# ducha-aiki/mods

Measured on AMD Instinct MI355X. Metric: image-pairs/sec (1024x768, HessAff+RootSIFT over the affine view ladder, MFMA FGINN match, LO-RANSAC H), higher is better.
Workload: dtype f32 (detect/describe) + u8 on the int8 matrix cores (distance matrix)

## Files before the change

include/modsx.h:

```cpp
#ifndef MODSX_H
#define MODSX_H
#include <stdint.h>
#ifdef __cplusplus
extern "C" {
#endif

#define MODSX_VERSION 100

typedef enum modsx_status {
  MODSX_OK = 0,
  MODSX_ERR_ARG = -1,
  MODSX_ERR_DEVICE = -2,
  MODSX_ERR_NOMEM = -3,
  MODSX_ERR_INTERNAL = -4,
  MODSX_ERR_CAPACITY = -5,
  MODSX_ERR_TIMEOUT = -6
} modsx_status;

enum { MODSX_FIXED_TH = 0, MODSX_RELATIVE_TH = 1, MODSX_FIXED_REG_NUMBER = 2, MODSX_RELATIVE_REG_NUMBER = 3,
       MODSX_NOT_LESS_THAN_REGIONS = 4 };
enum { MODSX_DET_HESSIAN = 0, MODSX_DET_DOG = 1, MODSX_DET_HARRIS = 2, MODSX_DET_MSER = 3 };
enum { MODSX_DESC_SIFT = 0, MODSX_DESC_ROOT_SIFT = 1, MODSX_DESC_HALF_SIFT = 2, MODSX_DESC_HALF_ROOT_SIFT = 3 };
#define MODSX_MAX_DESC 4
enum { MODSX_HESSIAN_DARK = 0, MODSX_HESSIAN_BRIGHT = 1, MODSX_HESSIAN_SADDLE = 2 };
// ... 178 lines not shown
                     const modsx_pair_params *par, modsx_pair_result *res);
void modsx_pair_result_release(modsx_pair_result *res);

int modsx_match_pairs(modsx_ctx *const *ctxs, int n_ctx, const modsx_image *const *imgs1,
                      const modsx_image *const *imgs2, int n_pairs, const modsx_pair_params *par,
                      modsx_pair_result *results);

int modsx_match_pairs_views(modsx_ctx *const *ctxs, int n_ctx, const modsx_image *const *imgs1,
                            const modsx_image *const *imgs2, int n_pairs, const modsx_view *views, int n_views,
                            const modsx_pair_params *par, modsx_pair_result *results);

int modsx_last_batch_verify(double *sum_ms, int *pairs, int *threads);
int modsx_last_match_geometry(int *qs, int *fat, int *S, int *tiles_per_split, int *ntiles_ub);
int modsx_describe_counters(modsx_ctx *ctx, long *out, int n);
int modsx_blur_geometry(const int *rows, const int *cols, int n, int *geometry);
int modsx_detect_counters(modsx_ctx *ctx, long *out, int n);
int modsx_debug_pyramids(modsx_ctx *ctx, const modsx_image *const *imgs, int n, const modsx_hessaff_params *par, int *geometry,
                         float *planes, unsigned long long cap_floats, unsigned long long *need_floats);
int modsx_debug_scan_levels(modsx_ctx *ctx, const float *resps, const float *blurs, int L, int rows, int cols,
                            const modsx_hessaff_params *par, modsx_candidate **cands, int *n_cands, modsx_sskp **out);
int modsx_debug_detect_scalespace_batch(modsx_ctx *ctx, const modsx_image *const *imgs, int n, const modsx_hessaff_params *par,
                                        modsx_sskp **out, int *counts);
int modsx_debug_orientation_counts(unsigned long long *launched, unsigned long long *skipped, int reset);
int modsx_debug_orientation_launches(unsigned long long *lds_table, unsigned long long *global_table, int reset);
int modsx_orientation_tables(unsigned char *bin_table, unsigned short *index_raster, float *weight_raster,
                             unsigned short *index_lanes, float *weight_lanes, int *counts);
int modsx_debug_reproject_certain_drop(const modsx_region *regs, int n, const double *H, int orig_w, int orig_h, double boxk,
                                       unsigned char *drop);
int modsx_debug_describe_plan(const modsx_region *regs, const int *counts, int nimages, double mr_size, int fast_extraction,
                              unsigned long long arena_floats, long *counters, int n, long *cuts, int cap_cuts, int *n_cuts);
// ... 233 lines not shown
```

mods_amd/__init__.py:

```python
import ctypes as C
import os
import subprocess

import numpy as np

_HERE = os.path.dirname(os.path.abspath(__file__))
LIB_PATH = os.environ.get("MODSX_LIB", os.path.join(_HERE, "libmodsx.so"))

KEYPOINT = np.dtype([("x", "f8"), ("y", "f8"), ("a11", "f8"), ("a12", "f8"), ("a21", "f8"), ("a22", "f8"),
                     ("s", "f8"), ("response", "f8"), ("octave_number", "i4"), ("pyramid_scale", "f8"),
                     ("sub_type", "i4")], align=True)
REGION = np.dtype([("img_id", "i4"), ("img_reproj_id", "i4"), ("id", "i4"), ("parent_id", "i4"), ("type", "i4"),
                   ("det_kp", KEYPOINT), ("reproj_kp", KEYPOINT)], align=True)
SSKP = np.dtype([("octave", "i4"), ("level", "i4"), ("r0", "i4"), ("c0", "i4"), ("r", "i4"), ("c", "i4"),
                 ("type", "i4"), ("pad", "i4"), ("b0", "f4"), ("b1", "f4"), ("b2", "f4"), ("val", "f4"),
                 ("x", "f4"), ("y", "f4"), ("s", "f4"), ("pixelDistance", "f4")], align=True)
TENT = np.dtype([("q", "i4"), ("t0", "i4"), ("tj", "i4"), ("t1", "i4"), ("d1", "f8"), ("d2", "f8"),
                 ("d2by2ndcl", "f8"), ("ratio", "f8")], align=True)
CANDIDATE = np.dtype([("img", "i4"), ("octave", "i4"), ("level", "i4"), ("type", "i4"), ("r0", "i4"), ("c0", "i4"), ("r", "i4"),
                      ("c", "i4"), ("b0", "f4"), ("b1", "f4"), ("b2", "f4"), ("val", "f4")], align=True)


class HessAffParams(C.Structure):
    _fields_ = [("threshold", C.c_float), ("mode", C.c_int), ("reg_number", C.c_int),
# ... 78 lines not shown
           "modsx_view_block_order", "modsx_detect_describe_views_sharded", "modsx_match_fginn_sharded",
           "modsx_match_pair_views_sharded", "modsx_match_pairs_views_sharded", "modsx_match_ladder_sharded", "modsx_comm_loopback_id", "modsx_comm_set_lanes",
           "modsx_comm_attach", "modsx_comm_lane_done", "modsx_comm_reset_lanes", "modsx_comm_set_timeout", "modsx_comm_stats",
           "modsx_shard_block_bytes", "modsx_shard_block_pack", "modsx_shard_blocks_unpack", "modsx_shard_device_pack",
           "modsx_shard_device_unpack", "modsx_verify_device_stats", "modsx_verify_device_timing", "modsx_comm_set_exchange",
           "modsx_shard_owner_plan", "modsx_db_create", "modsx_db_free", "modsx_db_rows", "modsx_db_nearest",
           "modsx_match_fginn_db", "modsx_match_fginn_db_device", "modsx_set_fginn_db",
           "modsx_debug_orientation_counts", "modsx_debug_orientation_launches", "modsx_orientation_tables",
           "modsx_debug_reproject_certain_drop", "modsx_debug_describe_plan",
           "modsx_debug_baumberg_geometry", "modsx_debug_baumberg_geometry_ctx", "modsx_debug_baumberg_variant",
           "modsx_debug_baumberg", "modsx_debug_check_borders", "modsx_debug_describe_lanes", "modsx_debug_describe_lane_map",
           "modsx_rep_create", "modsx_rep_free", "modsx_rep_add_views", "modsx_rep_append", "modsx_rep_class",
           "modsx_rep_match_fginn", "modsx_match_reps", "modsx_match_one_to_many",
           "modsx_match_hamming", "modsx_match_hamming_device", "modsx_hamming_tentatives", "modsx_debug_match_hamming",
           "modsx_match_regions_hamming", "modsx_debug_hamming_geometry",
           "modsx_blur_geometry", "modsx_detect_counters", "modsx_debug_pyramids", "modsx_debug_scan_levels",
           "modsx_debug_detect_scalespace_batch",
           "modsx_match_fginn_f32", "modsx_match_fginn_f32_device", "modsx_match_regions_f32", "modsx_debug_match_fginn_f32",
           "modsx_debug_fginn32_geometry", "modsx_debug_fginn32_dpass",
           "modsx_extract_patches", "modsx_extract_patches_device", "modsx_liop_patches", "modsx_liop_patches_device",
           "modsx_describe_regions_liop", "modsx_describe_regions_liop_device", "modsx_liop_tables", "modsx_debug_liop",
           "modsx_liop_counters",
           "modsx_describe_regions_raw", "modsx_describe_regions_raw_device", "modsx_sift_norm_rows", "modsx_sift_norm_rows_device",
           "modsx_describe_regions_dspsift", "modsx_describe_regions_dspsift_device", "modsx_dsp_counters",
           "modsx_surf_patches", "modsx_surf_patches_device", "modsx_describe_regions_surf", "modsx_describe_regions_surf_device",
           "modsx_surf_tables", "modsx_surf_counters",
           "modsx_detect_surf", "modsx_detect_surf_batch", "modsx_surf_regions", "modsx_surfdet_geometry", "modsx_surfdet_normalise",
           "modsx_debug_surfdet", "modsx_surfdet_counters",
           "modsx_daisy_dim", "modsx_daisy_patches", "modsx_daisy_patches_device", "modsx_describe_regions_daisy",
           "modsx_describe_regions_daisy_device", "modsx_daisy_tables", "modsx_daisy_counters"]
EXPORTS_DEGENSAC = ["exp_ransacHcustom", "exp_ransacFcustom", "HDs", "HDsi", "HDsidx", "HDsSym", "HDsiSym", "HDsSymidx",
# ... 68 lines not shown
        L.modsx_db_create.restype = C.c_void_p
        L.modsx_db_create.argtypes = [C.c_void_p, C.c_void_p, C.c_long, C.c_int]
        L.modsx_db_free.restype = None
        L.modsx_db_free.argtypes = [C.c_void_p, C.c_void_p]
        L.modsx_db_rows.restype = C.c_long
        L.modsx_db_rows.argtypes = [C.c_void_p]
        L.modsx_db_nearest.argtypes = [C.c_void_p, C.c_void_p, C.c_void_p, C.c_int, C.c_void_p]
        L.modsx_set_fginn_db.argtypes = [C.c_void_p, C.c_void_p]
        L.modsx_debug_reproject_certain_drop.argtypes = [C.c_void_p, C.c_int, C.c_void_p, C.c_int, C.c_int, C.c_double, C.c_void_p]
        L.modsx_describe_counters.argtypes = [C.c_void_p, C.c_void_p, C.c_int]
        L.modsx_debug_orientation_counts.argtypes = [C.c_void_p, C.c_void_p, C.c_int]
        L.modsx_debug_orientation_launches.argtypes = [C.c_void_p, C.c_void_p, C.c_int]
        L.modsx_orientation_tables.argtypes = [C.c_void_p] * 6
        L.modsx_blur_geometry.argtypes = [C.c_void_p, C.c_void_p, C.c_int, C.c_void_p]
        L.modsx_detect_counters.argtypes = [C.c_void_p, C.c_void_p, C.c_int]
        L.modsx_debug_pyramids.argtypes = [C.c_void_p, C.c_void_p, C.c_int, C.c_void_p, C.c_void_p, C.c_void_p, C.c_ulonglong,
                                           C.c_void_p]
        L.modsx_debug_scan_levels.argtypes = [C.c_void_p, C.c_void_p, C.c_void_p, C.c_int, C.c_int, C.c_int, C.c_void_p,
                                              C.c_void_p, C.c_void_p, C.c_void_p]
        L.modsx_debug_detect_scalespace_batch.argtypes = [C.c_void_p, C.c_void_p, C.c_int, C.c_void_p, C.c_void_p, C.c_void_p]
        L.modsx_debug_describe_plan.argtypes = [C.c_void_p, C.c_void_p, C.c_int, C.c_double, C.c_int, C.c_ulonglong, C.c_void_p, C.c_int,
                                                C.c_void_p, C.c_int, C.c_void_p]
        L.modsx_debug_baumberg_geometry.argtypes = [C.c_int, C.c_int, C.c_int, C.c_int, C.c_void_p]
        L.modsx_debug_baumberg.argtypes = [C.c_void_p, C.c_void_p, C.c_int, C.c_void_p, C.c_void_p, C.c_int, C.c_void_p, C.c_int, C.c_int,
                                           C.c_void_p, C.c_void_p, C.c_void_p, C.c_void_p, C.c_void_p]
        L.modsx_debug_baumberg_variant.argtypes = [C.c_int]
        L.modsx_debug_baumberg_geometry_ctx.argtypes = [C.c_void_p, C.c_int, C.c_int, C.c_int, C.c_int, C.c_void_p]
        L.modsx_debug_check_borders.argtypes = [C.c_void_p, C.c_int, C.c_void_p]
        L.modsx_debug_describe_lanes.argtypes = [C.c_int, C.c_void_p]
        L.modsx_debug_describe_lane_map.argtypes = [C.c_int, C.c_int, C.c_void_p, C.c_void_p, C.c_int]
# ... 460 lines not shown
        return C.c_void_p(self.h)

    def upload(self, pixels):
        a = np.ascontiguousarray(pixels)
        if a.dtype == np.uint8:
            dtype = 0
        else:
            a = np.ascontiguousarray(a, np.float32)
            dtype = 1
        ch = 1 if a.ndim == 2 else a.shape[2]
        h = lib().modsx_image_upload(self._c(), _p(a), a.shape[0], a.shape[1], ch, dtype)
        if not h:
            raise RuntimeError("modsx_image_upload failed: " + _err())
        return Image(self, h, a.shape[0], a.shape[1])

    def wrap_device(self, dev_ptr, rows, cols):
        h = lib().modsx_image_wrap_device(self._c(), C.c_void_p(dev_ptr), rows, cols)
        if not h:
            raise RuntimeError("modsx_image_wrap_device failed: " + _err())
        return Image(self, h, rows, cols)

    def synchronize(self):
        _check(lib().modsx_synchronize(self._c()), "synchronize")

    def gaussian_blur(self, img, sigma):
        out = np.empty((img.rows, img.cols), np.float32)
        _check(lib().modsx_gaussian_blur(self._c(), C.c_void_p(img.h), C.c_float(sigma), _p(out)), "gaussian_blur")
        return out

    def response(self, img, detector_type, norm):
# ... 253 lines not shown
        if out_ptr is not None:
            _check(lib().modsx_describe_regions_dspsift_device(*args, C.c_void_p(out_ptr)), "describe_regions_dspsift_device")
            return None
        desc = np.zeros((len(regs), 128), np.float32)
        _check(lib().modsx_describe_regions_dspsift(*args, _p(desc)), "describe_regions_dspsift")
        return desc

    def dsp_counters(self):
        return self._counters("modsx_dsp_counters", DSP_COUNTERS)

    def describe_counters(self):
        return self._counters("modsx_describe_counters", DESCRIBE_COUNTERS)

    def detect_counters(self):
        return self._counters("modsx_detect_counters", DETECT_COUNTERS)

    def debug_pyramids(self, images, params):
        n, L = len(images), params.numberOfScales + 2
        ptrs = (C.c_void_p * max(1, n))(*[im.h for im in images])
        geo = np.zeros((max(1, n), 49), np.int32)
        need = C.c_ulonglong(0)
        _check(lib().modsx_debug_pyramids(self._c(), ptrs, n, C.byref(params), _p(geo), None, 0, C.byref(need)), "debug_pyramids")
        planes = np.empty(max(1, need.value), np.float32)
        _check(lib().modsx_debug_pyramids(self._c(), ptrs, n, C.byref(params), _p(geo), _p(planes), need.value, C.byref(need)),
               "debug_pyramids")
        out, at = [], 0
        for i in range(n):
            octs = []
            for o in range(int(geo[i, 0])):
                r, c = int(geo[i, 1 + 2 * o]), int(geo[i, 2 + 2 * o])
# ... 364 lines not shown
def hamming_tentatives(nn2, distance_threshold):
    nn2 = np.ascontiguousarray(nn2, np.int32).reshape(-1, 4)
    out = C.c_void_p()
    n = _check(lib().modsx_hamming_tentatives(_p(nn2), len(nn2), C.c_double(distance_threshold), C.byref(out)), "hamming_tentatives")
    return _take(out, n, TENT)


def blur_geometry(shapes):
    sh = np.ascontiguousarray(shapes, np.int32).reshape(-1, 2)
    rows, cols = np.ascontiguousarray(sh[:, 0]), np.ascontiguousarray(sh[:, 1])
    geo = np.zeros(2, np.int32)
    _check(lib().modsx_blur_geometry(_p(rows), _p(cols), len(sh), _p(geo)), "blur_geometry")
    return int(geo[0]), int(geo[1])


FGINN32_GEOMETRY = ("tile", "splits", "workgroups", "DK", "tiles", "tiles_per_split")


def _f32_rows(d1, d2):
    d1, d2 = np.ascontiguousarray(d1, np.float32), np.ascontiguousarray(d2, np.float32)
    if d1.ndim != 2 or d2.ndim != 2 or d1.shape[1] != d2.shape[1]:
        raise ValueError("fginn_f32: two [n][dim] arrays of one width are expected")
    return d1, d2, d1.shape[1]


def fginn32_geometry(n1, n2, dim, splits=0):
    geo = np.zeros(6, np.int32)
    _check(lib().modsx_debug_fginn32_geometry(int(n1), int(n2), int(dim), int(splits), _p(geo)), "fginn32_geometry")
    return dict(zip(FGINN32_GEOMETRY, (int(x) for x in geo)))

# ... 270 lines not shown
```

mods_amd/csrc/capi.hip:

```cpp
#include <math.h>
#include <malloc.h>
#include <algorithm>
#include <atomic>
#include <chrono>
#include <mutex>
#include <thread>
#include <condition_variable>
#include <deque>
#include "engine_api.hpp"
#include "describe_plan.hpp"
#include "describe_lanes.hpp"

using namespace mx;

#define NEED(c)                                             \
  do {                                                      \
    if (!(c)) { mx::set_error("null argument: " #c); return MODSX_ERR_ARG; } \
  } while (0)

template <typename T>
static T *to_malloc(const std::vector<T> &v) {
  T *p = (T *)malloc(sizeof(T) * (v.size() ? v.size() : 1));
  if (p && !v.empty()) memcpy(p, v.data(), sizeof(T) * v.size());
  return p;
}

// ... 111 lines not shown
int modsx_image_update(modsx_ctx *ctx, modsx_image *im, const void *pixels, int rows, int cols, int channels, int dtype) {
  NEED(ctx); NEED(im); NEED(pixels);
  if ((channels != 1 && channels != 3) || (dtype != 0 && dtype != 1) || !im->owned || rows != im->rows || cols != im->cols) {
    mx::set_error("modsx_image_update: bad argument (the image must be an uploaded one of the same size)");
    return MODSX_ERR_ARG;
  }
  hipSetDevice(ctx->dev);
  const size_t n = (size_t)rows * cols, inBytes = n * channels * (dtype == 0 ? 1 : 4);
  if (!ctx->misc.ensure(inBytes)) return MODSX_ERR_NOMEM;
  if (hipMemcpyAsync(ctx->misc.p, pixels, inBytes, hipMemcpyHostToDevice, ctx->stream) != hipSuccess) { mx::set_error("image H2D copy failed"); return MODSX_ERR_DEVICE; }
  launch_gray(ctx->stream, ctx->misc.p, im->d, n, channels, dtype);
  if (hipStreamSynchronize(ctx->stream) != hipSuccess) { mx::set_error("image update sync failed"); return MODSX_ERR_DEVICE; }
  return MODSX_OK;
}

modsx_image *modsx_image_wrap_device(modsx_ctx *ctx, const float *dev_pixels, int rows, int cols) {
  if (!ctx || !dev_pixels || rows <= 0 || cols <= 0) { mx::set_error("modsx_image_wrap_device: bad argument"); return nullptr; }
  if (!image_size_ok(rows, cols)) return nullptr;
  modsx_image *im = new modsx_image();
  im->d = const_cast<float *>(dev_pixels); im->rows = rows; im->cols = cols; im->owned = false;
  return im;
}

void modsx_image_free(modsx_ctx *ctx, modsx_image *img) {
  if (!img) return;
  if (ctx) hipSetDevice(ctx->dev);
  if (img->owned && img->d) hipFree(img->d);
  delete img;
}

// ... 52 lines not shown
  if (!ctx->scratchA.ensure(npx * 4)) return MODSX_ERR_NOMEM;
  BlurBatch b;
  memset(&b, 0, sizeof b);
  int n = blur_ksize(sigma);
  if (n > MAX_TAPS) { mx::set_error("modsx_gaussian_blur: ksize > 17"); return MODSX_ERR_ARG; }
  if (n == 1) {
    MX_HIP(hipMemcpyAsync(out, img->d, npx * 4, hipMemcpyDeviceToHost, ctx->stream));
    MX_HIP(hipStreamSynchronize(ctx->stream));
    return MODSX_OK;
  }
  std::vector<float> k = gaussian_kernel(n, sigma);
  b.n = n;
  for (int i = 0; i < n; i++) b.k[i] = k[i];
  b.j[0].src = img->d; b.j[0].blur = (float *)ctx->scratchA.p; b.j[0].resp = nullptr; b.j[0].rows = img->rows;
  b.j[0].cols = img->cols; b.j[0].norm = 1.f;
  mx::book_blur(ctx, launch_blur_hess(ctx->stream, b, 1, img->rows, img->cols));
  MX_HIP(hipMemcpyAsync(out, ctx->scratchA.p, npx * 4, hipMemcpyDeviceToHost, ctx->stream));
  MX_HIP(hipStreamSynchronize(ctx->stream));
  MX_HIP(hipGetLastError());
  return MODSX_OK;
}

static int blur_any(modsx_ctx *c, const float *src, float *dst, float *tmp, float *dTaps, float *hTaps, int rows, int cols, float sigma) {
  const int n = blur_ksize(sigma);
  if (n == 1) { MX_HIP(hipMemcpyAsync(dst, src, (size_t)rows * cols * 4, hipMemcpyDeviceToDevice, c->stream)); return MODSX_OK; }
  const int nx = cols == 1 ? 1 : n, ny = rows == 1 ? 1 : n;
  std::vector<float> kx = gaussian_kernel(nx, sigma), ky = gaussian_kernel(ny, sigma);
  memcpy(hTaps, kx.data(), nx * 4); memcpy(hTaps + nx, ky.data(), ny * 4);
  MX_HIP(hipMemcpyAsync(dTaps, hTaps, (size_t)(nx + ny) * 4, hipMemcpyHostToDevice, c->stream));
  launch_blur_pass(c->stream, src, tmp, rows, cols, dTaps, nx, 0, 1);
  launch_blur_pass(c->stream, tmp, dst, rows, cols, dTaps + nx, ny, 1, 1);
// ... 201 lines not shown
  NEED(ctx);
  if (n < 0 || (n > 0 && !out)) { mx::set_error("modsx_describe_counters: bad argument"); return MODSX_ERR_ARG; }
  long sum[mx::DC_N] = {0};
  for (const modsx_ctx *head : {(const modsx_ctx *)ctx, (const modsx_ctx *)ctx->peer})
    for (const modsx_ctx *c = head; c; c = c->half)
      for (int q = 0; q < mx::DC_N; q++)
        if (q == mx::DC_MAX_CHUNKS) sum[q] = std::max(sum[q], c->descCnt[q]); else sum[q] += c->descCnt[q];
  for (int q = 0; q < n && q < mx::DC_N; q++) out[q] = sum[q];
  return mx::DC_N;
}

int modsx_blur_geometry(const int *rows, const int *cols, int n, int *geometry) {
  NEED(rows); NEED(cols); NEED(geometry);
  if (n < 1 || n > mx::MAXB) { mx::set_error("modsx_blur_geometry: 1 .. 32 planes"); return MODSX_ERR_ARG; }
  for (int i = 0; i < n; i++)
    if (rows[i] < 1 || cols[i] < 1 || !image_size_ok(rows[i], cols[i])) { mx::set_error("modsx_blur_geometry: plane size"); return MODSX_ERR_ARG; }
  const mx::BlurGeo g = mx::blur_geometry(rows, cols, n);
  geometry[0] = g.th; geometry[1] = g.tiles;
  return MODSX_OK;
}

int modsx_detect_counters(modsx_ctx *ctx, long *out, int n) {
  NEED(ctx);
  if (n < 0 || (n > 0 && !out)) { mx::set_error("modsx_detect_counters: bad argument"); return MODSX_ERR_ARG; }
  long sum[mx::DT_N] = {0};
  for (const modsx_ctx *head : {(const modsx_ctx *)ctx, (const modsx_ctx *)ctx->peer})
    for (const modsx_ctx *c = head; c; c = c->half)
      for (int q = 0; q < mx::DT_N; q++)
        if (q != mx::DT_LAST_JOBS && q != mx::DT_LAST_TILES && q != mx::DT_LAST_ACCEPTED) sum[q] += c->detCnt[q];
  for (int q : {(int)mx::DT_LAST_JOBS, (int)mx::DT_LAST_TILES, (int)mx::DT_LAST_ACCEPTED}) sum[q] = ctx->detCnt[q];
  for (int q = 0; q < n && q < mx::DT_N; q++) out[q] = sum[q];
  return mx::DT_N;
}
// ... 1213 lines not shown
```

mods_amd/csrc/engine.hpp:

```cpp
#pragma once
#include <hip/hip_runtime.h>
#include <stdint.h>
#include <stdlib.h>
#include <string.h>
#include <string>
#include <vector>
#include "../../include/modsx.h"
#include "kmath.hpp"

namespace mx {

#ifndef MODSX_MAXB
#define MODSX_MAXB 32
#endif
constexpr int MAXB = MODSX_MAXB;
constexpr int PAIR_GROUP = 4;
constexpr int NMS_MAXJ = 1024;
constexpr int MAX_TAPS = 17;

struct BlurJob {
  const float *src;
  float *blur;
  float *resp;
  int rows, cols;
  float norm;
  int pad;
};
struct BlurBatch {
  int n;
  float k[MAX_TAPS];
  BlurJob j[MAXB];
  int nj;
  int tile0[MAXB + 1];
};
struct ResizeJob {
  const float *src;
  float *dst;
  float *resp;
  int srows, scols, drows, dcols;
  float norm;
  int pad;
};
struct ResizeBatch { ResizeJob j[MAXB]; int nj; int tile0[MAXB + 1]; };
struct NmsJob {
  const float *low, *cur, *high, *blur;
  int rows, cols, img, octave, level, pad;
};
struct NmsBatch {
// ... 122 lines not shown
  } while (0)

std::vector<float> gaussian_kernel(int n, double sigma);
int blur_ksize(float sigma);
void gauss_mask(float *mask, int size);
void circular_gauss_mask(float *mask, int size, float sigma);
const double *atan_lut_host();
inline bool check_borders_host(int w, int h, float ofsx, float ofsy, float a11, float a12, float a21, float a22, int rw, int rh) {
  return check_borders(w, h, ofsx, ofsy, a11, a12, a21, a22, rw, rh);
}
bool invert3(const double *S, double *t);
void rectify(double &a11, double &a12, double &a21, double &a22);

struct BlurGeo { int th, tiles; };
BlurGeo blur_geometry(const int *rows, const int *cols, int n);
struct BlurLaunch { int th, tiles, R; };
BlurLaunch launch_blur_hess(hipStream_t s, const BlurBatch &b, int nj, int maxRows, int maxCols);
bool launch_hessian(hipStream_t s, const BlurBatch &b, int nj, int maxRows, int maxCols);
bool launch_resize_half(hipStream_t s, const ResizeBatch &b, int nj, int maxRows, int maxCols);
void launch_nms(hipStream_t s, const NmsBatch &b, const NmsJob *jobs, const int *tilePrefix, const int *tileJob, int nj,
                int nTiles, int4 *queue, unsigned *qcount, unsigned qcap, Candidate *out, unsigned *counter, unsigned cap,
                const int *octFirst = nullptr, int levelsPerOctave = 0);
size_t cand_sort_temp_bytes(unsigned nsort);
int launch_cand_order(hipStream_t s, const Candidate *cand, const unsigned *counter, unsigned nsort, unsigned long long *keys,
                      unsigned long long *keys2, unsigned *idx, unsigned *idx2, void *temp, size_t tempBytes, unsigned long long *tabKey,
                      unsigned *tabRank, unsigned tabSize, unsigned *slotOf, Candidate *out, unsigned *outCount);
constexpr int NMS_QUEUES = 64;
constexpr int NMS_TILE_ROWS = 16;
void launch_gray(hipStream_t s, const void *src, float *dst, size_t n, int channels, int dtype);
struct BaumGeo { int kernel, chunk, nchunks, grid; };
BaumGeo baumberg_geometry(int n, int W, int variant, int chunk, int resident = 0);
// ... 208 lines not shown
  unsigned short *dOriIdx = nullptr;
  float *dSiftMask = nullptr;
  unsigned short *dSiftMaskIdx = nullptr;
  int nSiftMask = 0;
  double *dAtan = nullptr;
  unsigned char *dOriBinTab = nullptr;
  float *dSiftOTab = nullptr;
  int *dSiftBins = nullptr;
  double *dSiftW = nullptr;
  double timings[6];
  mx::Profiler prof;
  size_t lastCandCount = 0;
  const mx::DbSet *fginnDb = nullptr;
  long descCnt[mx::DC_N] = {0};
  long detCnt[mx::DT_N] = {0};
  double hammingMs[2] = {0, 0};
  double fginn32Ms[2] = {0, 0};
  mx::DevBuf patchBuf, patchOut;
  mx::DevBuf liopTab, liopDbg, liopCnt;
  long liopCounters[4] = {0, 0, 0, 0};
  mx::DevBuf dspRows;
  long dspCounters[3] = {0, 0, 0};
  static constexpr int SURF_TABS = 4;
  mx::DevBuf surfTab[SURF_TABS];
  double surfTabMr[SURF_TABS] = {0, 0, 0, 0};
  int surfTabNext = 0;
  long surfCounters[3] = {0, 0, 0};
  static constexpr int DAISY_TABS = 4;
  mx::DevBuf daisyTab[DAISY_TABS];
  int daisyTabKey[DAISY_TABS] = {0, 0, 0, 0};
  int daisyTabNext = 0;
  long daisyCounters[3] = {0, 0, 0};
  mx::DevBuf sdInteg, sdResp, sdLap, sdFlags, sdCounts, sdTab, sdPoints, sdExt;
  mx::PinBuf sdHost, sdBack;
  long sdCounters[5] = {0, 0, 0, 0, 0};
  int busyDepth = 0;
  int shardLane = 0;
  modsx_ctx *peer = nullptr;
  modsx_ctx *half = nullptr;
  mx::DevBuf halfDesc[4];
  void *worker = nullptr;
};

namespace mx {
inline void book_blur(modsx_ctx *c, const BlurLaunch &g) {
  if (!g.th) return;
  c->detCnt[g.th == 32 ? DT_BLUR_TH32 : DT_BLUR_TH16]++;
  c->detCnt[DT_BLUR_R1 + g.R - 1]++;
}
}
```

mods_amd/csrc/engine_detect.hip:

```cpp
#include <math.h>
#include <algorithm>
#include <mutex>
#include <dlfcn.h>
#include <string>
#include "engine_api.hpp"

namespace mx {

static int cv_round(double v) { return (int)lrint(v); }

struct SigmaPlan {
  int levels;
  float sigmaStep;
  float curSigma[8];
  float incSigma[8];
};

static SigmaPlan make_sigma_plan(const modsx_hessaff_params &p) {
  SigmaPlan s;
  s.levels = p.numberOfScales + 2;
  s.sigmaStep = powf(2.0f, 1.0f / (float)p.numberOfScales);
  float cur = p.initialSigma;
  s.curSigma[0] = cur; s.incSigma[0] = 0;
  for (int i = 1; i < s.levels; i++) {
// ... 68 lines not shown
    float sigma = sqrtf(p.initialSigma * p.initialSigma - curSigma0 * curSigma0);
    int rc = fill_taps(bb, sigma);
    if (rc) return rc;
  }
  for (int k = 0; k < lv.n; k++) {
    const int i = lv.img[k];
    Octave &oc = c->pyr[i].oct[0];
    BlurJob &j = bb.j[k];
    j.src = imgs[i]->d; j.blur = oc.blur[0]; j.resp = hess ? oc.resp[0] : nullptr; j.rows = oc.rows; j.cols = oc.cols;
    j.norm = sp.curSigma[0] * sp.curSigma[0];
    if (!preBlur) {
      MX_HIP(hipMemcpyAsync(oc.blur[0], imgs[i]->d, (size_t)oc.rows * oc.cols * 4, hipMemcpyDeviceToDevice, s));
      j.src = oc.blur[0];
    }
  }
  if (preBlur) { ProfScope ps(c, K_BLUR_HESS, lv.px * 12); book_blur(c, launch_blur_hess(s, bb, lv.n, lv.mr, lv.mc)); }
  else if (hess) { ProfScope ps(c, K_HESSIAN, lv.px * 8); c->detCnt[DT_HESSIAN] += launch_hessian(s, bb, lv.n, lv.mr, lv.mc); }
  return MODSX_OK;
}

static void launch_resize_level(modsx_ctx *c, const LiveOctave &lv, int o, const modsx_hessaff_params &p, const SigmaPlan &sp, bool hess) {
  ResizeBatch rb;
  memset(&rb, 0, sizeof rb);
  double spx = 0;
  for (int k = 0; k < lv.n; k++) {
    Octave &pv = c->pyr[lv.img[k]].oct[o - 1], &oc = c->pyr[lv.img[k]].oct[o];
    ResizeJob &r = rb.j[k];
    r.src = pv.blur[p.numberOfScales]; r.dst = oc.blur[0];
    r.srows = pv.rows; r.scols = pv.cols; r.drows = oc.rows; r.dcols = oc.cols;
    r.resp = hess ? oc.resp[0] : nullptr; r.norm = sp.curSigma[0] * sp.curSigma[0];
    spx += (double)pv.rows * pv.cols;
// ... 50 lines not shown
      }
    }
  }
  return MODSX_OK;
}

int build_pyramids(modsx_ctx *c, const modsx_image *const *imgs, int n, const modsx_hessaff_params &p,
                   bool singleOctaveFromFirstLevel) {
  if (n <= 0 || n > MAXB) { set_error("batch size"); return MODSX_ERR_ARG; }
  if (p.numberOfScales < 1 || p.numberOfScales > 6) { set_error("numberOfScales"); return MODSX_ERR_ARG; }
  if (p.border < 1) { set_error("border must be at least 1"); return MODSX_ERR_ARG; }
  if (p.detectorType != MODSX_DET_HESSIAN && p.detectorType != MODSX_DET_DOG && p.detectorType != MODSX_DET_HARRIS) {
    set_error("detectorType must be Hessian (0), DoG (1) or Harris (2)");
    return MODSX_ERR_ARG;
  }
  const bool hess = p.detectorType == MODSX_DET_HESSIAN;
  const SigmaPlan sp = make_sigma_plan(p);
  int maxOct = 0;
  int rc = plan_octaves(c, imgs, n, sp.levels, 2 * p.border + 2, singleOctaveFromFirstLevel, &maxOct);
  if (rc) return rc;
  for (int o = 0; o < maxOct; o++) {
    const LiveOctave lv = live_octave(c, n, o);
    if (o == 0) rc = launch_first_level(c, imgs, lv, p, sp, hess, singleOctaveFromFirstLevel);
    else launch_resize_level(c, lv, o, p, sp, hess);
    if (rc) return rc;
    for (int l = 1; l < sp.levels; l++) {
      BlurBatch b2;
      memset(&b2, 0, sizeof b2);
      rc = fill_taps(b2, sp.incSigma[l]);
      if (rc) return rc;
      for (int k = 0; k < lv.n; k++) {
        Octave &oc = c->pyr[lv.img[k]].oct[o];
        BlurJob &j = b2.j[k];
        j.src = oc.blur[l - 1]; j.blur = oc.blur[l]; j.resp = hess ? oc.resp[l] : nullptr; j.rows = oc.rows; j.cols = oc.cols;
        j.norm = sp.curSigma[l] * sp.curSigma[l];
      }
      ProfScope ps(c, K_BLUR_HESS, lv.px * 12);
      book_blur(c, launch_blur_hess(c->stream, b2, lv.n, lv.mr, lv.mc));
    }
    if (!hess) rc = launch_other_responses(c, lv, o, p, sp);
    if (rc) return rc;
  }
  MX_HIP(hipGetLastError());
  return MODSX_OK;
}

static const unsigned CAND_CAP = 1u << 21;

static NmsBatch nms_thresholds(const modsx_hessaff_params &p) {
  NmsBatch nb;
  memset(&nb, 0, sizeof nb);
  nb.edgeScoreThreshold = (p.edgeEigenValueRatio + 1.0f) * (p.edgeEigenValueRatio + 1.0f) / p.edgeEigenValueRatio;
  float finalTh = p.threshold;
// ... 520 lines not shown
```

mods_amd/csrc/kernels_pyramid.hip:

```cpp
#include "engine.hpp"

namespace mx {

constexpr int TW = 64;
constexpr int TMP_W = TW + 4;

MX_D int find_job(const int *tile0, int nj, int t) {
  int j = 0;
  while (j + 1 < nj && t >= tile0[j + 1]) j++;
  return j;
}

typedef float f2 __attribute__((ext_vector_type(2)));

template <int R, int TH>
__global__ __launch_bounds__(256) void k_blur_hess(BlurBatch batch) {
  constexpr int BLR_H = TH + 4;
  const int ji = find_job(batch.tile0, batch.nj, blockIdx.x);
  const BlurJob jb = batch.j[ji];
  const int rows = jb.rows, cols = jb.cols;
  const int lt = blockIdx.x - batch.tile0[ji], ntx = (cols + TW - 1) / TW;
  const int tx0 = (lt % ntx) * TW, ty0 = (lt / ntx) * TH;
  constexpr int n = 2 * R + 1;
  constexpr int sh = BLR_H + 2 * R, sw = TMP_W + 2 * R;
// ... 71 lines not shown
    const float *B = blr + (ly + 1) * TMP_W + (lx + 1);
    const unsigned gofs = __umul24((unsigned)gy, (unsigned)cols) + (unsigned)gx;
    jb.blur[gofs] = B[0];
    if (jb.resp) {
      float o = 0.f;
      if (gy >= 1 && gy < rows - 1 && gx >= 1 && gx < cols - 1) {
        const float v11 = B[-TMP_W - 1], v12 = B[-TMP_W], v13 = B[-TMP_W + 1];
        const float v21 = B[-1], v22 = B[0], v23 = B[1];
        const float v31 = B[TMP_W - 1], v32 = B[TMP_W], v33 = B[TMP_W + 1];
        float Lxx = (v21 - 2 * v22 + v23);
        float Lyy = (v12 - 2 * v22 + v32);
        float Lxy = (v13 - v11 + v31 - v33) / 4.0f;
        o = (Lxx * Lyy - Lxy * Lxy) * norm2;
      }
      jb.resp[gofs] = o;
    }
  }
}

__global__ __launch_bounds__(256) void k_hessian(BlurBatch batch) {
  const int ji = find_job(batch.tile0, batch.nj, blockIdx.x);
  const BlurJob jb = batch.j[ji];
  const int rows = jb.rows, cols = jb.cols;
  const int lt = blockIdx.x - batch.tile0[ji], ntx = (cols + 63) / 64;
  const int gx = (lt % ntx) * 64 + (threadIdx.x & 63), gy = (lt / ntx) * 4 + (threadIdx.x >> 6);
  if (gx >= cols || gy >= rows) return;
  float o = 0.f;
  if (gy >= 1 && gy < rows - 1 && gx >= 1 && gx < cols - 1) {
    const float *B = jb.src + (size_t)gy * cols + gx;
    const float v11 = B[-cols - 1], v12 = B[-cols], v13 = B[-cols + 1];
// ... 355 lines not shown
    case 6: hipLaunchKernelGGL((k_blur_hess<6, TH>), grid, dim3(256), 0, s, b); break;
    case 7: hipLaunchKernelGGL((k_blur_hess<7, TH>), grid, dim3(256), 0, s, b); break;
    default: hipLaunchKernelGGL((k_blur_hess<8, TH>), grid, dim3(256), 0, s, b); break;
  }
}
BlurGeo blur_geometry(const int *rows, const int *cols, int n) {
  auto tiles = [&](int th) {
    int t = 0;
    for (int i = 0; i < n; i++) t += ((cols[i] + TW - 1) / TW) * ((rows[i] + th - 1) / th);
    return t;
  };
  const int t32 = tiles(32);
  if (t32 >= 2560) return {32, t32};
  return {16, tiles(16)};
}
BlurLaunch launch_blur_hess(hipStream_t s, const BlurBatch &bin, int nj, int, int) {
  BlurBatch b = bin;
  int rows[MAXB], cols[MAXB];
  for (int i = 0; i < nj; i++) { rows[i] = b.j[i].rows; cols[i] = b.j[i].cols; }
  const BlurGeo g = blur_geometry(rows, cols, nj);
  if (g.tiles <= 0) return {0, 0, 0};
  const int tiles = fill_tiles(b, nj, TW, g.th);
  if (g.th == 32) launch_blur_hess_th<32>(s, b, tiles);
  else launch_blur_hess_th<16>(s, b, tiles);
  const int R = b.n >> 1;
  return {g.th, tiles, R >= 1 && R <= 7 ? R : 8};
}
bool launch_hessian(hipStream_t s, const BlurBatch &bin, int nj, int, int) {
  BlurBatch b = bin;
  const int tiles = fill_tiles(b, nj, 64, 4);
  if (tiles > 0) hipLaunchKernelGGL(k_hessian, dim3(tiles), dim3(256), 0, s, b);
  return tiles > 0;
}
bool launch_resize_half(hipStream_t s, const ResizeBatch &bin, int nj, int, int) {
  ResizeBatch b = bin;
  b.nj = nj;
  int t = 0;
  for (int i = 0; i < nj; i++) { b.tile0[i] = t; t += ((b.j[i].dcols + 63) / 64) * ((b.j[i].drows + 3) / 4); }
  b.tile0[nj] = t;
  if (t > 0) MX_DUP(K_RESIZE) hipLaunchKernelGGL(k_resize_half, dim3(t), dim3(256), 0, s, b);
  return t > 0;
// ... 146 lines not shown
```

Baseline: 236.4.

## Add strip-walking blur+Hessian kernel that reuses vertical halo across stacked tiles

Adds a k_blur_hess_strip kernel in which each workgroup walks a vertical strip of several 32-row tiles. It carries the separable blur's vertical halo rows forward in shared memory instead of reloading and re-filtering them per tile, and prefetches the next tile's source into registers while the current one is filtered. The Hessian output is computed over 4-row register windows, and only live columns are processed. The path is on by default for the TH=32 geometry, with env overrides for the strip length. Longer strips mean fewer workgroups, which risks lower occupancy and load balance on the GPU.

```diff
diff --git a/include/modsx.h b/include/modsx.h
--- a/include/modsx.h
+++ b/include/modsx.h
@@ -216,6 +216,9 @@
 int modsx_last_match_geometry(int *qs, int *fat, int *S, int *tiles_per_split, int *ntiles_ub);
 int modsx_describe_counters(modsx_ctx *ctx, long *out, int n);
 int modsx_blur_geometry(const int *rows, const int *cols, int n, int *geometry);
+int modsx_blur_strip_geometry(const int *rows, const int *cols, int n, int *geometry);
+int modsx_debug_blur_strips(modsx_ctx *ctx, long *launches, long *strips);
+modsx_image *modsx_debug_upload_plane(modsx_ctx *ctx, const float *pixels, int rows, int cols);
 int modsx_detect_counters(modsx_ctx *ctx, long *out, int n);
 int modsx_debug_pyramids(modsx_ctx *ctx, const modsx_image *const *imgs, int n, const modsx_hessaff_params *par, int *geometry,
                          float *planes, unsigned long long cap_floats, unsigned long long *need_floats);
diff --git a/mods_amd/__init__.py b/mods_amd/__init__.py
--- a/mods_amd/__init__.py
+++ b/mods_amd/__init__.py
@@ -116,7 +116,7 @@
            "modsx_rep_match_fginn", "modsx_match_reps", "modsx_match_one_to_many",
            "modsx_match_hamming", "modsx_match_hamming_device", "modsx_hamming_tentatives", "modsx_debug_match_hamming",
            "modsx_match_regions_hamming", "modsx_debug_hamming_geometry",
-           "modsx_blur_geometry", "modsx_detect_counters", "modsx_debug_pyramids", "modsx_debug_scan_levels",
+           "modsx_blur_geometry", "modsx_blur_strip_geometry", "modsx_debug_blur_strips", "modsx_debug_upload_plane", "modsx_detect_counters", "modsx_debug_pyramids", "modsx_debug_scan_levels",
            "modsx_debug_detect_scalespace_batch",
            "modsx_match_fginn_f32", "modsx_match_fginn_f32_device", "modsx_match_regions_f32", "modsx_debug_match_fginn_f32",
            "modsx_debug_fginn32_geometry", "modsx_debug_fginn32_dpass",
@@ -215,6 +215,10 @@
         L.modsx_orientation_tables.argtypes = [C.c_void_p] * 6
         L.modsx_blur_geometry.argtypes = [C.c_void_p, C.c_void_p, C.c_int, C.c_void_p]
         L.modsx_detect_counters.argtypes = [C.c_void_p, C.c_void_p, C.c_int]
+        L.modsx_blur_strip_geometry.argtypes = [C.c_void_p, C.c_void_p, C.c_int, C.c_void_p]
+        L.modsx_debug_blur_strips.argtypes = [C.c_void_p, C.c_void_p, C.c_void_p]
+        L.modsx_debug_upload_plane.restype = C.c_void_p
+        L.modsx_debug_upload_plane.argtypes = [C.c_void_p, C.c_void_p, C.c_int, C.c_int]
         L.modsx_debug_pyramids.argtypes = [C.c_void_p, C.c_void_p, C.c_int, C.c_void_p, C.c_void_p, C.c_void_p, C.c_ulonglong,
                                            C.c_void_p]
         L.modsx_debug_scan_levels.argtypes = [C.c_void_p, C.c_void_p, C.c_void_p, C.c_int, C.c_int, C.c_int, C.c_void_p,
@@ -705,6 +709,15 @@
             raise RuntimeError("modsx_image_upload failed: " + _err())
         return Image(self, h, a.shape[0], a.shape[1])
 
+    def upload_plane(self, plane):
+        a = np.ascontiguousarray(plane, np.float32)
+        if a.ndim != 2:
+            raise ValueError("upload_plane: a 2-D array is expected")
+        h = lib().modsx_debug_upload_plane(self._c(), _p(a), a.shape[0], a.shape[1])
+        if not h:
+            raise RuntimeError("modsx_debug_upload_plane failed: " + _err())
+        return Image(self, h, a.shape[0], a.shape[1])
+
     def wrap_device(self, dev_ptr, rows, cols):
         h = lib().modsx_image_wrap_device(self._c(), C.c_void_p(dev_ptr), rows, cols)
         if not h:
@@ -988,6 +1001,11 @@
 
     def detect_counters(self):
         return self._counters("modsx_detect_counters", DETECT_COUNTERS)
+
+    def debug_blur_strips(self):
+        launches, strips = C.c_long(0), C.c_long(0)
+        _check(lib().modsx_debug_blur_strips(self._c(), C.byref(launches), C.byref(strips)), "debug_blur_strips")
+        return int(launches.value), int(strips.value)
 
     def debug_pyramids(self, images, params):
         n, L = len(images), params.numberOfScales + 2
@@ -1382,6 +1400,14 @@
     return int(geo[0]), int(geo[1])
 
 
+def blur_strip_geometry(shapes):
+    sh = np.ascontiguousarray(shapes, np.int32).reshape(-1, 2)
+    rows, cols = np.ascontiguousarray(sh[:, 0]), np.ascontiguousarray(sh[:, 1])
+    geo = np.zeros(3, np.int32)
+    _check(lib().modsx_blur_strip_geometry(_p(rows), _p(cols), len(sh), _p(geo)), "blur_strip_geometry")
+    return int(geo[0]), int(geo[1]), int(geo[2])
+
+
 FGINN32_GEOMETRY = ("tile", "splits", "workgroups", "DK", "tiles", "tiles_per_split")
 
 
diff --git a/mods_amd/csrc/blur_strips.hpp b/mods_amd/csrc/blur_strips.hpp
--- /dev/null
+++ b/mods_amd/csrc/blur_strips.hpp
@@ -0,0 +1,28 @@
+#pragma once
+
+namespace mx {
+
+struct BlurStripGeo { int ls, strips, tiles; };
+
+constexpr int BLUR_STRIP_TH = 32, BLUR_STRIP_TW = 64;
+constexpr int BLUR_STRIP_SLOTS = 1280;
+inline int blur_strip_length(int tiles32) {
+  const int cand[5] = {8, 6, 4, 3, 2};
+  for (int c : cand)
+    if (tiles32 >= c * BLUR_STRIP_SLOTS) return c;
+  return 2;
+}
+inline int blur_strips_of(int rows, int cols, int ls) {
+  const int ntx = (cols + BLUR_STRIP_TW - 1) / BLUR_STRIP_TW, nty = (rows + BLUR_STRIP_TH - 1) / BLUR_STRIP_TH;
+  return ntx * ((nty + ls - 1) / ls);
+}
+inline BlurStripGeo blur_strip_geometry(const int *rows, const int *cols, int n, int lsForce = 0) {
+  BlurStripGeo g = {0, 0, 0};
+  for (int i = 0; i < n; i++)
+    g.tiles += ((cols[i] + BLUR_STRIP_TW - 1) / BLUR_STRIP_TW) * ((rows[i] + BLUR_STRIP_TH - 1) / BLUR_STRIP_TH);
+  g.ls = lsForce > 0 ? lsForce : blur_strip_length(g.tiles);
+  for (int i = 0; i < n; i++) g.strips += blur_strips_of(rows[i], cols[i], g.ls);
+  return g;
+}
+
+}
diff --git a/mods_amd/csrc/capi.hip b/mods_amd/csrc/capi.hip
--- a/mods_amd/csrc/capi.hip
+++ b/mods_amd/csrc/capi.hip
@@ -10,6 +10,7 @@
 #include "engine_api.hpp"
 #include "describe_plan.hpp"
 #include "describe_lanes.hpp"
+#include "blur_strips.hpp"
 
 using namespace mx;
 
@@ -151,6 +152,24 @@
   return MODSX_OK;
 }
 
+static bool plane_size_ok(int rows, int cols) {
+  return rows >= 2 && cols >= 2 && rows <= (1 << 20) && cols <= (1 << 20) && (long long)rows * cols <= (1ll << 26);
+}
+
+modsx_image *modsx_debug_upload_plane(modsx_ctx *ctx, const float *pixels, int rows, int cols) {
+  if (!ctx || !pixels) { mx::set_error("modsx_debug_upload_plane: bad argument"); return nullptr; }
+  if (!plane_size_ok(rows, cols)) { mx::set_error("modsx_debug_upload_plane: 2 .. 2^20 px per side and at most 64 Mpx"); return nullptr; }
+  hipSetDevice(ctx->dev);
+  const size_t n = (size_t)rows * cols;
+  modsx_image *im = new modsx_image();
+  im->rows = rows; im->cols = cols; im->owned = true; im->d = nullptr;
+  if (hipMalloc(&im->d, n * 4) != hipSuccess) { mx::set_error("hipMalloc plane"); delete im; return nullptr; }
+  if (hipMemcpyAsync(im->d, pixels, n * 4, hipMemcpyHostToDevice, ctx->stream) != hipSuccess || hipStreamSynchronize(ctx->stream) != hipSuccess) {
+    mx::set_error("plane H2D copy failed"); hipFree(im->d); delete im; return nullptr;
+  }
+  return im;
+}
+
 modsx_image *modsx_image_wrap_device(modsx_ctx *ctx, const float *dev_pixels, int rows, int cols) {
   if (!ctx || !dev_pixels || rows <= 0 || cols <= 0) { mx::set_error("modsx_image_wrap_device: bad argument"); return nullptr; }
   if (!image_size_ok(rows, cols)) return nullptr;
@@ -233,7 +252,8 @@
   for (int i = 0; i < n; i++) b.k[i] = k[i];
   b.j[0].src = img->d; b.j[0].blur = (float *)ctx->scratchA.p; b.j[0].resp = nullptr; b.j[0].rows = img->rows;
   b.j[0].cols = img->cols; b.j[0].norm = 1.f;
-  mx::book_blur(ctx, launch_blur_hess(ctx->stream, b, 1, img->rows, img->cols));
+  const int brc = mx::book_blur(ctx, launch_blur_hess(ctx->stream, b, 1, img->rows, img->cols));
+  if (brc) return brc;
   MX_HIP(hipMemcpyAsync(out, ctx->scratchA.p, npx * 4, hipMemcpyDeviceToHost, ctx->stream));
   MX_HIP(hipStreamSynchronize(ctx->stream));
   MX_HIP(hipGetLastError());
@@ -465,9 +485,28 @@
   NEED(rows); NEED(cols); NEED(geometry);
   if (n < 1 || n > mx::MAXB) { mx::set_error("modsx_blur_geometry: 1 .. 32 planes"); return MODSX_ERR_ARG; }
   for (int i = 0; i < n; i++)
-    if (rows[i] < 1 || cols[i] < 1 || !image_size_ok(rows[i], cols[i])) { mx::set_error("modsx_blur_geometry: plane size"); return MODSX_ERR_ARG; }
+    if (!plane_size_ok(rows[i], cols[i])) { mx::set_error("modsx_blur_geometry: plane size"); return MODSX_ERR_ARG; }
   const mx::BlurGeo g = mx::blur_geometry(rows, cols, n);
   geometry[0] = g.th; geometry[1] = g.tiles;
+  return MODSX_OK;
+}
+
+int modsx_blur_strip_geometry(const int *rows, const int *cols, int n, int *geometry) {
+  NEED(rows); NEED(cols); NEED(geometry);
+  if (n < 1 || n > mx::MAXB) { mx::set_error("modsx_blur_strip_geometry: 1 .. 32 planes"); return MODSX_ERR_ARG; }
+  for (int i = 0; i < n; i++)
+    if (!plane_size_ok(rows[i], cols[i])) { mx::set_error("modsx_blur_strip_geometry: plane size"); return MODSX_ERR_ARG; }
+  const mx::BlurStripGeo g = mx::blur_strip_geometry(rows, cols, n);
+  geometry[0] = g.ls; geometry[1] = g.strips; geometry[2] = g.tiles;
+  return MODSX_OK;
+}
+
+int modsx_debug_blur_strips(modsx_ctx *ctx, long *launches, long *strips) {
+  NEED(ctx); NEED(launches); NEED(strips);
+  long sum[2] = {0, 0};
+  for (const modsx_ctx *head : {(const modsx_ctx *)ctx, (const modsx_ctx *)ctx->peer})
+    for (const modsx_ctx *c = head; c; c = c->half) { sum[0] += c->stripCnt[0]; sum[1] += c->stripCnt[1]; }
+  *launches = sum[0]; *strips = sum[1];
   return MODSX_OK;
 }
 
diff --git a/mods_amd/csrc/engine.hpp b/mods_amd/csrc/engine.hpp
--- a/mods_amd/csrc/engine.hpp
+++ b/mods_amd/csrc/engine.hpp
@@ -32,6 +32,7 @@
   BlurJob j[MAXB];
   int nj;
   int tile0[MAXB + 1];
+  int ls;
 };
 struct ResizeJob {
   const float *src;
@@ -184,7 +185,7 @@
 
 struct BlurGeo { int th, tiles; };
 BlurGeo blur_geometry(const int *rows, const int *cols, int n);
-struct BlurLaunch { int th, tiles, R; };
+struct BlurLaunch { int th, tiles, R, strips; };
 BlurLaunch launch_blur_hess(hipStream_t s, const BlurBatch &b, int nj, int maxRows, int maxCols);
 bool launch_hessian(hipStream_t s, const BlurBatch &b, int nj, int maxRows, int maxCols);
 bool launch_resize_half(hipStream_t s, const ResizeBatch &b, int nj, int maxRows, int maxCols);
@@ -423,6 +424,7 @@
   const mx::DbSet *fginnDb = nullptr;
   long descCnt[mx::DC_N] = {0};
   long detCnt[mx::DT_N] = {0};
+  long stripCnt[2] = {0, 0};
   double hammingMs[2] = {0, 0};
   double fginn32Ms[2] = {0, 0};
   mx::DevBuf patchBuf, patchOut;
@@ -452,9 +454,12 @@
 };
 
 namespace mx {
-inline void book_blur(modsx_ctx *c, const BlurLaunch &g) {
-  if (!g.th) return;
+inline int book_blur(modsx_ctx *c, const BlurLaunch &g) {
+  if (g.th < 0) { set_error("blur launch: a plane is blurred in place (src aliases blur or resp)"); return MODSX_ERR_ARG; }
+  if (!g.th) return MODSX_OK;
   c->detCnt[g.th == 32 ? DT_BLUR_TH32 : DT_BLUR_TH16]++;
   c->detCnt[DT_BLUR_R1 + g.R - 1]++;
-}
-}
+  if (g.strips > 0) { c->stripCnt[0]++; c->stripCnt[1] += g.strips; }
+  return MODSX_OK;
+}
+}
diff --git a/mods_amd/csrc/engine_detect.hip b/mods_amd/csrc/engine_detect.hip
--- a/mods_amd/csrc/engine_detect.hip
+++ b/mods_amd/csrc/engine_detect.hip
@@ -106,7 +106,7 @@
       j.src = oc.blur[0];
     }
   }
-  if (preBlur) { ProfScope ps(c, K_BLUR_HESS, lv.px * 12); book_blur(c, launch_blur_hess(s, bb, lv.n, lv.mr, lv.mc)); }
+  if (preBlur) { ProfScope ps(c, K_BLUR_HESS, lv.px * 12); const int rc = book_blur(c, launch_blur_hess(s, bb, lv.n, lv.mr, lv.mc)); if (rc) return rc; }
   else if (hess) { ProfScope ps(c, K_HESSIAN, lv.px * 8); c->detCnt[DT_HESSIAN] += launch_hessian(s, bb, lv.n, lv.mr, lv.mc); }
   return MODSX_OK;
 }
@@ -187,6 +187,11 @@
     set_error("detectorType must be Hessian (0), DoG (1) or Harris (2)");
     return MODSX_ERR_ARG;
   }
+  for (int i = 0; i < n; i++)
+    if (!singleOctaveFromFirstLevel && (imgs[i]->rows > 16384 || imgs[i]->cols > 16384)) {
+      set_error("a plane larger than 16384 px per side serves modsx_gaussian_blur and modsx_octave_levels only");
+      return MODSX_ERR_ARG;
+    }
   const bool hess = p.detectorType == MODSX_DET_HESSIAN;
   const SigmaPlan sp = make_sigma_plan(p);
   int maxOct = 0;
@@ -209,7 +214,8 @@
         j.norm = sp.curSigma[l] * sp.curSigma[l];
       }
       ProfScope ps(c, K_BLUR_HESS, lv.px * 12);
-      book_blur(c, launch_blur_hess(c->stream, b2, lv.n, lv.mr, lv.mc));
+      rc = book_blur(c, launch_blur_hess(c->stream, b2, lv.n, lv.mr, lv.mc));
+      if (rc) return rc;
     }
     if (!hess) rc = launch_other_responses(c, lv, o, p, sp);
     if (rc) return rc;
diff --git a/mods_amd/csrc/kernels_pyramid.hip b/mods_amd/csrc/kernels_pyramid.hip
--- a/mods_amd/csrc/kernels_pyramid.hip
+++ b/mods_amd/csrc/kernels_pyramid.hip
@@ -1,4 +1,5 @@
 #include "engine.hpp"
+#include "blur_strips.hpp"
 
 namespace mx {
 
@@ -109,6 +110,206 @@
         o = (Lxx * Lyy - Lxy * Lxy) * norm2;
       }
       jb.resp[gofs] = o;
+    }
+  }
+}
+
+#ifndef MODSX_STRIP_PREFETCH
+#define MODSX_STRIP_PREFETCH 1
+#endif
+#ifndef MODSX_STRIP_LIVE_COLS
+#define MODSX_STRIP_LIVE_COLS 1
+#endif
+#ifndef MODSX_STRIP_WINDOW4
+#define MODSX_STRIP_WINDOW4 1
+#endif
+typedef float __attribute__((address_space(1))) *gfloat_p;
+
+MX_D unsigned strip_magic(unsigned d) { return 65536u / d + 1u; }
+MX_D int strip_div(int i, unsigned m) { return (int)(__umul24((unsigned)i, m) >> 16); }
+
+template <int R, int NR>
+MX_D void strip_load(gcfloat_p img, int rows, int cols, int y0, int x0, int tid, float (&t)[(NR * (TMP_W + 2 * R) + 255) / 256]) {
+  constexpr int sw = TMP_W + 2 * R, PER = (NR * sw + 255) / 256;
+#pragma unroll
+  for (int u = 0; u < PER; u++) {
+    const int i = tid + 256 * u, ii = i < NR * sw ? i : NR * sw - 1;
+    const int ly = ii / sw, lx = ii - ly * sw;
+    int gy = y0 + ly, gx = x0 + lx;
+    gy = gy < 0 ? 0 : (gy > rows - 1 ? rows - 1 : gy);
+    gx = gx < 0 ? 0 : (gx > cols - 1 ? cols - 1 : gx);
+    t[u] = img[__umul24((unsigned)gy, (unsigned)cols) + (unsigned)gx];
+  }
+}
+template <int R, int NR>
+MX_D void strip_park(float *src, int tid, const float (&t)[(NR * (TMP_W + 2 * R) + 255) / 256]) {
+  constexpr int sw = TMP_W + 2 * R, SW = (sw + 3) & ~3, PER = (NR * sw + 255) / 256;
+#pragma unroll
+  for (int u = 0; u < PER; u++) {
+    const int i = tid + 256 * u;
+    if (i < NR * sw) { const int ly = i / sw, lx = i - ly * sw; src[(ly >> 1) * (2 * SW) + 2 * lx + (ly & 1)] = t[u]; }
+  }
+}
+template <int R>
+MX_D void strip_rowpass(const float *src, float *tmp, const float *k, int tid, int npairs, int row0, int ng, unsigned mg) {
+  constexpr int n = 2 * R + 1, SW = (TMP_W + 2 * R + 3) & ~3;
+  for (int i = tid; i < npairs * ng; i += 256) {
+    const int lp = strip_div(i, mg), g = i - lp * ng;
+    const f2 *S = reinterpret_cast<const f2 *>(src) + lp * SW + 4 * g;
+    f2 w[4 + 2 * R];
+#pragma unroll
+    for (int q = 0; q < (4 + 2 * R) / 2; q++) {
+      const float4 t = *reinterpret_cast<const float4 *>(S + 2 * q);
+      w[2 * q] = (f2){t.x, t.y}; w[2 * q + 1] = (f2){t.z, t.w};
+    }
+    f2 v[4];
+#pragma unroll
+    for (int o = 0; o < 4; o++) {
+      if (n <= 5) {
+        v[o] = w[o + R] * k[R];
+#pragma unroll
+        for (int j = 1; j <= R; j++) v[o] = v[o] + (w[o + R - j] + w[o + R + j]) * k[R + j];
+      } else {
+        v[o] = (f2){0.f, 0.f};
+#pragma unroll
+        for (int j = 0; j < n; j++) v[o] = v[o] + w[o + j] * k[j];
+      }
+    }
+    *reinterpret_cast<float4 *>(tmp + (row0 + 2 * lp) * TMP_W + 4 * g) = make_float4(v[0].x, v[1].x, v[2].x, v[3].x);
+    *reinterpret_cast<float4 *>(tmp + (row0 + 2 * lp + 1) * TMP_W + 4 * g) = make_float4(v[0].y, v[1].y, v[2].y, v[3].y);
+  }
+}
+
+template <int R>
+__global__ __launch_bounds__(256) __attribute__((amdgpu_waves_per_eu(R <= 6 ? 7 : 6))) void k_blur_hess_strip(BlurBatch batch) {
+  constexpr int TH = 32, BLR_H = TH + 4, KEEP = 4 + 2 * R;
+  constexpr int sh = BLR_H + 2 * R, sw = TMP_W + 2 * R, SW = (sw + 3) & ~3;
+  static_assert(KEEP <= TH && KEEP % 2 == 0, "the top halo is one batch of row pairs that fits src");
+  constexpr int SRC_F = TH * SW > BLR_H * TMP_W ? TH * SW : BLR_H * TMP_W;
+  __shared__ __attribute__((aligned(16))) float src[SRC_F];
+  __shared__ __attribute__((aligned(16))) float tmp[sh * TMP_W];
+  float *blr = src;
+  const int nstrips = batch.tile0[batch.nj];
+  const int si = xcd_chunk(blockIdx.x, nstrips);
+  if (si >= nstrips) return;
+  const int ji = find_job(batch.tile0, batch.nj, si);
+  const BlurJob jb = batch.j[ji];
+  const int rows = jb.rows, cols = jb.cols, tid = threadIdx.x;
+  const int ls = si - batch.tile0[ji], ntx = (cols + TW - 1) / TW, nty = (rows + TH - 1) / TH;
+  const int sy = ls / ntx, tx0 = (ls - sy * ntx) * TW;
+  const int tyFirst = sy * batch.ls, ntile = min(batch.ls, nty - tyFirst);
+  const gcfloat_p img = as_global(jb.src);
+  const gfloat_p oblur = (gfloat_p)jb.blur, oresp = (gfloat_p)jb.resp;
+  const int live = min(TW, cols - tx0);
+#if MODSX_STRIP_LIVE_COLS
+  const int ng = (live + 2 + 3) >> 2, np = (live + 2 + 1) >> 1;
+#else
+  const int ng = TMP_W / 4, np = TMP_W / 2;
+#endif
+  const unsigned mg = strip_magic((unsigned)ng), mp = strip_magic((unsigned)np);
+  const float norm2 = jb.norm * jb.norm;
+  int ty0 = tyFirst * TH;
+  float t[(TH * sw + 255) / 256];
+  strip_load<R, TH>(img, rows, cols, ty0 + 3 + R, tx0 - 1 - R, tid, t);
+  {
+    float h[(KEEP * sw + 255) / 256];
+    strip_load<R, KEEP>(img, rows, cols, ty0 - 1 - R, tx0 - 1 - R, tid, h);
+    strip_park<R, KEEP>(src, tid, h);
+    __syncthreads();
+    strip_rowpass<R>(src, tmp, batch.k, tid, KEEP / 2, 0, ng, mg);
+    __syncthreads();
+  }
+  for (int kt = 0; kt < ntile; kt++, ty0 += TH) {
+    int tl = tid;
+    asm volatile("" : "+v"(tl));
+    strip_park<R, TH>(src, tl, t);
+    __syncthreads();
+#if MODSX_STRIP_PREFETCH == 1
+    if (kt + 1 < ntile) strip_load<R, TH>(img, rows, cols, ty0 + TH + 3 + R, tx0 - 1 - R, tl, t);
+#endif
+    strip_rowpass<R>(src, tmp, batch.k, tid, TH / 2, KEEP, ng, mg);
+    __syncthreads();
+    for (int i = tid; i < (BLR_H / 4) * np; i += 256) {
+      const int gy = strip_div(i, mp), lx = 2 * (i - gy * np);
+      const float *S = tmp + (4 * gy) * TMP_W + lx;
+      f2 w[4 + 2 * R];
+#pragma unroll
+      for (int q = 0; q < 4 + 2 * R; q++) w[q] = *reinterpret_cast<const f2 *>(S + q * TMP_W);
+#pragma unroll
+      for (int o = 0; o < 4; o++) {
+        f2 v = w[o + R] * batch.k[R] + (f2){0.f, 0.f};
+#pragma unroll
+        for (int j = 1; j <= R; j++) v = v + (w[o + R + j] + w[o + R - j]) * batch.k[R + j];
+        *reinterpret_cast<f2 *>(blr + (4 * gy + o) * TMP_W + lx) = v;
+      }
+    }
+    __syncthreads();
+#if MODSX_STRIP_PREFETCH == 2
+    if (kt + 1 < ntile) strip_load<R, TH>(img, rows, cols, ty0 + TH + 3 + R, tx0 - 1 - R, tl, t);
+#endif
+    if (kt + 1 < ntile)
+      for (int i = tid; i < KEEP * (TMP_W / 4); i += 256)
+        reinterpret_cast<float4 *>(tmp)[i] = reinterpret_cast<const float4 *>(tmp)[TH * (TMP_W / 4) + i];
+    const int rl = min(TH, rows - ty0);
+#if MODSX_STRIP_WINDOW4
+    const int ngr = (rl + 3) >> 2;
+    const unsigned mv = strip_magic((unsigned)live);
+    for (int i = tid; i < ngr * live; i += 256) {
+      const int gq = strip_div(i, mv), lx = i - gq * live;
+      const int ly0 = 4 * gq, gx = tx0 + lx;
+      float w[6][3];
+#pragma unroll
+      for (int r = 0; r < 6; r++) {
+        const float *B = blr + (ly0 + r) * TMP_W + lx;
+        w[r][0] = B[0]; w[r][1] = B[1]; w[r][2] = B[2];
+      }
+      const bool colIn = gx >= 1 && gx < cols - 1;
+      unsigned gofs = __umul24((unsigned)(ty0 + ly0), (unsigned)cols) + (unsigned)gx;
+#pragma unroll
+      for (int q = 0; q < 4; q++, gofs += (unsigned)cols) {
+        if (ly0 + q >= rl) break;
+        const int gy = ty0 + ly0 + q;
+        oblur[gofs] = w[q + 1][1];
+        if (jb.resp) {
+          const float v11 = w[q][0], v12 = w[q][1], v13 = w[q][2];
+          const float v21 = w[q + 1][0], v22 = w[q + 1][1], v23 = w[q + 1][2];
+          const float v31 = w[q + 2][0], v32 = w[q + 2][1], v33 = w[q + 2][2];
+          float Lxx = (v21 - 2 * v22 + v23);
+          float Lyy = (v12 - 2 * v22 + v32);
+          float Lxy = (v13 - v11 + v31 - v33) / 4.0f;
+          const float h = (Lxx * Lyy - Lxy * Lxy) * norm2;
+          oresp[gofs] = (colIn && gy >= 1 && gy < rows - 1) ? h : 0.f;
+        }
+      }
+    }
+#else
+    for (int i = tid; i < TH * TW; i += 256) {
+      const int ly = i / TW, lx = i - ly * TW;
+      const int gy = ty0 + ly, gx = tx0 + lx;
+      if (ly >= rl || gx >= cols) continue;
+      const float *B = blr + (ly + 1) * TMP_W + (lx + 1);
+      const unsigned gofs = __umul24((unsigned)gy, (unsigned)cols) + (unsigned)gx;
+      oblur[gofs] = B[0];
+      if (jb.resp) {
+        float o = 0.f;
+        if (gy >= 1 && gy < rows - 1 && gx >= 1 && gx < cols - 1) {
+          const float v11 = B[-TMP_W - 1], v12 = B[-TMP_W], v13 = B[-TMP_W + 1];
+          const float v21 = B[-1], v22 = B[0], v23 = B[1];
+          const float v31 = B[TMP_W - 1], v32 = B[TMP_W], v33 = B[TMP_W + 1];
+          float Lxx = (v21 - 2 * v22 + v23);
+          float Lyy = (v12 - 2 * v22 + v32);
+          float Lxy = (v13 - v11 + v31 - v33) / 4.0f;
+          o = (Lxx * Lyy - Lxy * Lxy) * norm2;
+        }
+        oresp[gofs] = o;
+      }
+    }
+#endif
+    if (kt + 1 < ntile) {
+#if !MODSX_STRIP_PREFETCH
+      strip_load<R, TH>(img, rows, cols, ty0 + TH + 3 + R, tx0 - 1 - R, tl, t);
+#endif
+      __syncthreads();
     }
   }
 }
@@ -494,17 +695,49 @@
   if (t32 >= 2560) return {32, t32};
   return {16, tiles(16)};
 }
+static bool blur_strips_on() {
+  static const bool on = !(getenv("MODSX_BLUR_STRIPS") && atoi(getenv("MODSX_BLUR_STRIPS")) == 0);
+  return on;
+}
+static int blur_strip_ls_forced() {
+  static const int ls = getenv("MODSX_BLUR_STRIP_LS") ? atoi(getenv("MODSX_BLUR_STRIP_LS")) : 0;
+  return ls >= 1 && ls <= 1024 ? ls : 0;
+}
+static void launch_blur_hess_strips(hipStream_t s, const BlurBatch &b, int strips) {
+  dim3 grid(8 * ((strips + 7) / 8));
+  MX_DUP(K_BLUR_HESS) switch (b.n >> 1) {
+    case 1: hipLaunchKernelGGL(k_blur_hess_strip<1>, grid, dim3(256), 0, s, b); break;
+    case 2: hipLaunchKernelGGL(k_blur_hess_strip<2>, grid, dim3(256), 0, s, b); break;
+    case 3: hipLaunchKernelGGL(k_blur_hess_strip<3>, grid, dim3(256), 0, s, b); break;
+    case 4: hipLaunchKernelGGL(k_blur_hess_strip<4>, grid, dim3(256), 0, s, b); break;
+    case 5: hipLaunchKernelGGL(k_blur_hess_strip<5>, grid, dim3(256), 0, s, b); break;
+    case 6: hipLaunchKernelGGL(k_blur_hess_strip<6>, grid, dim3(256), 0, s, b); break;
+    case 7: hipLaunchKernelGGL(k_blur_hess_strip<7>, grid, dim3(256), 0, s, b); break;
+    default: hipLaunchKernelGGL(k_blur_hess_strip<8>, grid, dim3(256), 0, s, b); break;
+  }
+}
 BlurLaunch launch_blur_hess(hipStream_t s, const BlurBatch &bin, int nj, int, int) {
   BlurBatch b = bin;
   int rows[MAXB], cols[MAXB];
   for (int i = 0; i < nj; i++) { rows[i] = b.j[i].rows; cols[i] = b.j[i].cols; }
   const BlurGeo g = blur_geometry(rows, cols, nj);
-  if (g.tiles <= 0) return {0, 0, 0};
+  if (g.tiles <= 0) return {0, 0, 0, 0};
+  const int R = b.n >> 1, Rk = R >= 1 && R <= 7 ? R : 8;
+  for (int i = 0; i < nj; i++)
+    if (b.j[i].src == b.j[i].blur || b.j[i].src == b.j[i].resp) return {-1, 0, 0, 0};
+  if (g.th == 32 && blur_strips_on()) {
+    const BlurStripGeo sg = blur_strip_geometry(rows, cols, nj, blur_strip_ls_forced());
+    b.nj = nj; b.ls = sg.ls;
+    int t = 0;
+    for (int i = 0; i < nj; i++) { b.tile0[i] = t; t += blur_strips_of(rows[i], cols[i], sg.ls); }
+    b.tile0[nj] = t;
+    launch_blur_hess_strips(s, b, t);
+    return {32, g.tiles, Rk, t};
+  }
   const int tiles = fill_tiles(b, nj, TW, g.th);
   if (g.th == 32) launch_blur_hess_th<32>(s, b, tiles);
   else launch_blur_hess_th<16>(s, b, tiles);
-  const int R = b.n >> 1;
-  return {g.th, tiles, R >= 1 && R <= 7 ? R : 8};
+  return {g.th, tiles, Rk, 0};
 }
 bool launch_hessian(hipStream_t s, const BlurBatch &bin, int nj, int, int) {
   BlurBatch b = bin;
```

Result: no change. 237.9, median of 6 (+0.7%).
